# yunfanye/Bittorrent-with-Congestion-Control

Hardware: AMD Instinct MI355X
Metric: GiB/s SHA-1 hashed (device-resident 512KiB chunks) at 1/2/4/8 MI355X (higher is better)
Workload: dtype u32

## Files before the change

### bittorrent-with-congestion-control_amd/btsha1.py

```python
import ctypes
import os

HERE = os.path.dirname(os.path.abspath(__file__))
LIB_PATH = os.environ.get("BT_SHA1_LIB", os.path.join(HERE, "libbtsha1.so"))
CHUNK = 512 * 1024
DIGEST = 20


class BtSha1Error(RuntimeError):
    pass


if not os.path.exists(LIB_PATH):
    raise ImportError(f"libbtsha1.so not built at {LIB_PATH}: run `make` (or __graft_entry__.build())")
lib = ctypes.CDLL(LIB_PATH)

_u8p = ctypes.POINTER(ctypes.c_uint8)
_vp = ctypes.c_void_p
_u64 = ctypes.c_uint64
_i64 = ctypes.c_int64


class Verdict(ctypes.Structure):
    _fields_ = [("tag", ctypes.c_uint64), ("ok", ctypes.c_int32), ("digest", ctypes.c_uint8 * 20)]
# ... 31 lines not shown
_sig("bt_sha1_last_error", ctypes.c_char_p)
_sig("bt_sha1_build_info", ctypes.c_char_p)
_sig("bt_sha1_set_ring_depth", ctypes.c_int, ctypes.c_int)
_sig("bt_sha1_set_variant", ctypes.c_int, ctypes.c_int, ctypes.c_int, ctypes.c_int)
_sig("bt_sha1_set_latency_batch", _u64, _u64)
_sig("bt_sha1_set_seglist_latency_batch", _u64, _u64)
_sig("bt_sha1_seglist_kernel_name", ctypes.c_char_p, _u64)
_sig("bt_sha1_chunks_dev", ctypes.c_int, _vp, _u64, _u64, _u64, _vp, _vp)
_sig("bt_sha1_verify_dev", ctypes.c_int, _vp, _u64, _u64, _u64, _vp, _vp, _vp, _vp)
_sig("bt_sha1_column_dev", ctypes.c_int, _vp, _u64, _u64, _u64, ctypes.c_int, _vp, _u64, _vp, _vp, _vp, _vp)
_sig("bt_sha1_ragged_dev", ctypes.c_int, _vp, _vp, _vp, _u64, _vp, _vp)
_sig("bt_sha1_ragged_verify_dev", ctypes.c_int, _vp, _vp, _vp, _u64, _vp, _vp, _vp, _vp)
_sig("bt_sha1_fill_synthetic", ctypes.c_int, _vp, _u64, _u64, _u64, _vp)
_sig("bt_sha1_chunks_host", _i64, _vp, _u64, _u64, _vp)
_sig("bt_sha1_host_register", ctypes.c_int, _vp, _u64)
_sig("bt_sha1_host_unregister", ctypes.c_int, _vp)
_sig("bt_sha1_chunks_host_multi", _i64, _vp, _u64, _u64, _vp, ctypes.c_int)
_sig("bt_sha1_chunks_host_devices", _i64, _vp, _u64, _u64, _vp, ctypes.POINTER(ctypes.c_int), ctypes.c_int)
_sig("bt_sha1_source_id", ctypes.c_char_p)
_sig("bt_sha1_set_chain_batch", _u64, _u64)
_sig("bt_sha1_kernel_name", ctypes.c_char_p, _u64)
_sig("bt_sha1_clock_probe", ctypes.c_int, _vp, _u64, _u64, _u64, _vp, _vp, _vp)
_sig("bt_sha1_wallclock_khz", _i64)
_sig("bt_sha1_debug_barrier_stats", ctypes.c_int, ctypes.POINTER(ctypes.c_uint64), ctypes.c_int)
_sig("bt_sha1_debug_dropin_residue", _i64, ctypes.c_int)
_sig("bt_sha1_chunks_file", _i64, _vp, _u64, _vp, _u64)
_sig("bt_sha1_get_pipeline_stats", ctypes.c_int, ctypes.POINTER(PipelineStats))
_sig("bt_sha1_set_pageable_feed", ctypes.c_int, ctypes.c_int)
_sig("bt_sha1_verifier_create", _vp, ctypes.c_int, ctypes.c_uint32, ctypes.c_uint32, ctypes.c_uint32)
_sig("bt_sha1_verifier_destroy", None, _vp)
_sig("bt_sha1_verifier_slot", _vp, _vp)
_sig("bt_sha1_verifier_commit", ctypes.c_int, _vp, _vp, ctypes.c_uint32, _vp, _u64)
_sig("bt_sha1_verifier_release", ctypes.c_int, _vp, _vp)
_sig("bt_sha1_verifier_submit", ctypes.c_int, _vp, _vp, ctypes.c_uint32, _vp, _u64)
_sig("bt_sha1_verifier_flush", ctypes.c_int, _vp)
_sig("bt_sha1_verifier_poll", ctypes.c_int, _vp, ctypes.POINTER(Verdict), ctypes.c_int)
_sig("bt_sha1_verifier_drain", ctypes.c_int, _vp, ctypes.POINTER(Verdict), ctypes.c_int)
_sig("bt_sha1_verifier_pending", _i64, _vp)


class VerifierStats(ctypes.Structure):
    _fields_ = [(f, ctypes.c_uint64) for f in ("batches", "ragged_batches", "chunks", "short_chunks", "released")]


_sig("bt_sha1_verifier_create_ragged", _vp, ctypes.c_int, ctypes.c_uint32, ctypes.c_uint32, ctypes.c_uint32)
_sig("bt_sha1_verifier_get_stats", ctypes.c_int, _vp, ctypes.POINTER(VerifierStats))


class Seg(ctypes.Structure):
    _fields_ = [("off", ctypes.c_uint64), ("len", ctypes.c_uint32), ("reserved", ctypes.c_uint32)]


class VerifierGatherStats(ctypes.Structure):
    _fields_ = [(f, ctypes.c_uint64) for f in ("gather_batches", "gather_chunks", "segments", "payload_bytes",
                                               "copied_bytes")]


_sig("bt_sha1_gather_dev", ctypes.c_int, _vp, _vp, _vp, _vp, _u64, _vp, _vp)
_sig("bt_sha1_gather_verify_dev", ctypes.c_int, _vp, _vp, _vp, _vp, _u64, _vp, _vp, _vp, _vp)
_sig("bt_sha1_set_segchain_batch", _u64, _u64)


class PktGeom(ctypes.Structure):
    _fields_ = [(f, ctypes.c_uint32) for f in ("stride", "header", "payload", "slot_pkts")]


# ... 400 lines not shown
            self.h = lib.bt_sha1_verifier_create_gather(device, chunk_len, max_segs, batch, nstreams)
        else:
            create = lib.bt_sha1_verifier_create_ragged if ragged else lib.bt_sha1_verifier_create
            self.h = create(device, chunk_len, batch, nstreams)
        if not self.h:
            kind = "_gather" if gather else "_ragged" if ragged else ""
            raise BtSha1Error(f"bt_sha1_verifier_create{kind}: {last_error()}")
        self.chunk_len = chunk_len
        self.ragged = ragged
        self.gather = gather
        self.max_segs = max_segs

    def submit(self, chunk, expected, tag):
        buf, n = _host_buf(chunk)
        e = (ctypes.c_uint8 * 20).from_buffer_copy(bytes(expected))
        _check(lib.bt_sha1_verifier_submit(self.h, buf, n, e, tag), "bt_sha1_verifier_submit")

    def slot(self):
        p = lib.bt_sha1_verifier_slot(self.h)
        if not p:
            raise BtSha1Error(f"bt_sha1_verifier_slot: {last_error()}")
        return p

    def commit(self, slot, expected, tag, length=None):
        e = (ctypes.c_uint8 * 20).from_buffer_copy(bytes(expected))
        _check(lib.bt_sha1_verifier_commit(self.h, slot, length or self.chunk_len, e, tag),
               "bt_sha1_verifier_commit")

    def commit_gather(self, slot, segs, expected, tag):
        e = (ctypes.c_uint8 * 20).from_buffer_copy(bytes(expected))
        table = (Seg * max(len(segs), 1))(*[Seg(off, length, 0) for off, length in segs])
        _check(lib.bt_sha1_verifier_commit_gather(self.h, slot, table, len(segs), e, tag),
               "bt_sha1_verifier_commit_gather")

    def release(self, slot):
        _check(lib.bt_sha1_verifier_release(self.h, slot), "bt_sha1_verifier_release")

    def flush(self):
        _check(lib.bt_sha1_verifier_flush(self.h), "bt_sha1_verifier_flush")

    def slot_fill(self, chunk, expected, tag):
        p = self.slot()
        ctypes.memmove(p, bytes(chunk), len(chunk))
        self.commit(p, expected, tag, len(chunk))

    def _collect(self, fn, max_n=4096):
        out = (Verdict * max_n)()
        got = _check(fn(self.h, out, max_n), "verifier")
        return [(out[i].tag, bool(out[i].ok), bytes(out[i].digest)) for i in range(got)]

    def poll(self):
        return self._collect(lib.bt_sha1_verifier_poll)

    def drain(self):
        res = []
        while True:
            r = self._collect(lib.bt_sha1_verifier_drain)
            if not r:
                return res
            res += r

    def pending(self):
        return lib.bt_sha1_verifier_pending(self.h)

    def stats(self):
        s = VerifierStats()
# ... 230 lines not shown
```

### bittorrent-with-congestion-control_amd/csrc/bt_runtime.cpp

```cpp
#include "bt_runtime.h"

#include <cstdarg>
#include <memory>
#include <vector>

namespace btsha1 {

thread_local std::string t_err;
__thread int t_dev = 0;
std::atomic<int> g_variant{310};

void set_err(const char *fmt, ...) {
  char buf[512];
  va_list ap;
  va_start(ap, fmt);
  vsnprintf(buf, sizeof buf, fmt, ap);
  va_end(ap);
  t_err = buf;
}

[[noreturn]] void die(const char *where) {
  fprintf(stderr, "libbtsha1: %s: %s\n", where, t_err.c_str());
  fflush(stderr);
  abort();
}

bool trace_on() {
  static const bool on = [] {
    const char *e = getenv("BT_SHA1_TRACE");
    return e && *e && *e != '0';
  }();
  return on;
}

namespace {
std::mutex g_ctx_mu;
std::vector<std::unique_ptr<DevCtx>> g_ctx;
}

int device_count() {
  int n = 0;
  if (hipGetDeviceCount(&n) != hipSuccess) return 0;
  return n;
}

DevCtx *ctx_for(int dev) {
  std::lock_guard<std::mutex> g(g_ctx_mu);
  int n = device_count();
  if (n <= 0) {
    set_err("no HIP device visible (hipGetDeviceCount = 0)");
    return nullptr;
// ... 593 lines not shown
```

### bittorrent-with-congestion-control_amd/csrc/bt_runtime.h

```cpp
#pragma once
#include <hip/hip_runtime.h>

#include <algorithm>
#include <atomic>
#include <chrono>
#include <cstdio>
#include <cstdlib>
#include <cstring>
#include <functional>
#include <mutex>
#include <string>

#include <sched.h>

#include "bt_sha1.h"
#include "sha1_launch.h"

namespace btsha1 __attribute__((visibility("hidden"))) {

extern thread_local std::string t_err;
extern __thread int t_dev;
extern std::atomic<int> g_variant;

void set_err(const char *fmt, ...);

#define BT_CK(expr)                                                                  \
  do {                                                                               \
    hipError_t e_ = (expr);                                                          \
    if (e_ != hipSuccess) {                                                          \
      set_err("%s failed: %s (%s:%d)", #expr, hipGetErrorString(e_), __FILE__, __LINE__); \
      return -1;                                                                     \
    }                                                                                \
  } while (0)

[[noreturn]] void die(const char *where);

struct KeepDevice {
  int prev = -1;
  KeepDevice() {
    if (hipGetDevice(&prev) != hipSuccess) prev = -1;
  }
  ~KeepDevice() {
    int cur = -1;
    if (prev >= 0 && hipGetDevice(&cur) == hipSuccess && cur != prev) (void)hipSetDevice(prev);
  }
  KeepDevice(const KeepDevice &) = delete;
  KeepDevice &operator=(const KeepDevice &) = delete;
};

constexpr uint32_t kMaxColumns = 16;

struct DevBuf {
  void *p = nullptr;
  size_t cap = 0;
  int ensure(size_t need) {
    if (need <= cap) return 0;
    if (p) (void)hipFree(p);
    p = nullptr;
    cap = 0;
    size_t sz = std::max<size_t>(need, 4096);
    BT_CK(hipMalloc(&p, sz));
    cap = sz;
    return 0;
  }
  void release() {
// ... 99 lines not shown
```

### bittorrent-with-congestion-control_amd/csrc/bt_verifier.cpp

```cpp
#include "bt_columns.h"
#include "bt_runtime.h"

#include <deque>
#include <vector>

using namespace btsha1;

struct VBatch {
  hipStream_t s = nullptr;
  hipEvent_t ev = nullptr;
  hipStream_t hs = nullptr;
  hipEvent_t cev[kMaxColumns] = {};
  uint32_t *d_state = nullptr;
  StageBuf slots;
  uint8_t *h_in = nullptr, *h_exp = nullptr, *h_ok = nullptr, *h_dig = nullptr;
  uint64_t *h_off = nullptr;
  uint32_t *h_len = nullptr;
  bt_sha1_seg *h_segs = nullptr;
  uint64_t *h_first = nullptr;
  uint32_t *h_count = nullptr;
  uint8_t *d_in = nullptr;
  std::vector<uint64_t> tags;
  std::vector<uint8_t> state;
  uint32_t reserved = 0, settled = 0;
  bool closed = false, inflight = false;
};

struct bt_sha1_verifier {
  int dev = 0;
  uint32_t chunk_len = 0, batch = 0;
  uint32_t pitch = 0;
  bool ragged = false;
  bool gather = false;
  uint32_t max_segs = 0;
  bt_sha1_verifier_stats st = {};
  bt_sha1_verifier_gather_stats gs = {};
  std::vector<VBatch> b;
  uint32_t fill = 0;
  std::deque<uint32_t> order;
  std::deque<bt_sha1_verdict> done;
  int64_t queued = 0;
};

namespace {

int v_harvest(bt_sha1_verifier *v, VBatch &b) {
  BT_CK(hipEventSynchronize(b.ev));
  for (uint32_t i = 0; i < b.reserved; ++i) {
    if (b.state[i] != 2) continue;
    bt_sha1_verdict r;
    r.tag = b.tags[i];
    r.ok = b.h_ok[i] ? 1 : 0;
    memcpy(r.digest, b.h_dig + 20 * i, 20);
    v->done.push_back(r);
  }
  std::fill(b.state.begin(), b.state.end(), 0);
  b.reserved = b.settled = 0;
  b.closed = b.inflight = false;
  return 0;
}

uint32_t v_columns(uint64_t chunk_len, uint64_t rows) {
  const uint32_t parts = split_columns(chunk_len);
  return parts && rows >= 2 && rows * chunk_len >= column_min_bytes() ? parts : 0;
}

int v_launch_columns(bt_sha1_verifier *v, VBatch &b, uint32_t parts) {
  const uint64_t cl = v->chunk_len, rows = b.reserved, w = cl / parts;
  if (!b.hs) BT_CK(hipStreamCreateWithFlags(&b.hs, hipStreamNonBlocking));
  if (!b.d_state) BT_CK(hipMalloc((void **)&b.d_state, 20 * (size_t)v->batch));
  const ColumnRun run{b.s, b.hs, b.cev, parts, rows, w, cl, b.d_in, b.d_state};
  for (uint32_t j = 0; j < parts; ++j) {
    BT_CK(hipMemcpy2DAsync(b.d_in + j * rows * w, (size_t)w, b.h_in + j * w, (size_t)cl, (size_t)w, (size_t)rows,
                           hipMemcpyHostToDevice, b.s));
    const bool last = j + 1 == parts;
    if (hash_column(run, j, last ? b.h_dig : nullptr, last ? b.h_exp : nullptr, last ? b.h_ok : nullptr)) return -1;
  }
  BT_CK(hipEventRecord(b.ev, b.hs));
  return 0;
}

bool v_needs_ragged(const bt_sha1_verifier *v, const VBatch &b) {
  if (!v->ragged) return false;
  if (v->pitch != v->chunk_len) return true;
  for (uint32_t i = 0; i < b.reserved; ++i)
    if (b.state[i] == 2 && b.h_len[i] != v->chunk_len) return true;
  return false;
}

int v_launch(bt_sha1_verifier *v, uint32_t idx) {
  VBatch &b = v->b[idx];
  if (b.reserved == 0) {
    b.closed = false;
    return 0;
  }
  ++v->st.batches;
  if (v->gather) {
    const size_t bytes = (size_t)b.reserved * v->pitch;
    ++v->gs.gather_batches;
    v->gs.copied_bytes += bytes;
    BT_CK(hipMemcpyAsync(b.d_in, b.h_in, bytes, hipMemcpyHostToDevice, b.s));
    BT_CK(btsha1_launch_gather(b.d_in, b.h_segs, b.h_first, b.h_count, b.reserved, b.h_dig, b.h_exp, b.h_ok, b.s));
    BT_CK(hipEventRecord(b.ev, b.s));
    b.inflight = true;
    v->order.push_back(idx);
    return 0;
  }
  if (v_needs_ragged(v, b)) {
    ++v->st.ragged_batches;
    BT_CK(hipMemcpyAsync(b.d_in, b.h_in, (size_t)b.reserved * v->pitch, hipMemcpyHostToDevice, b.s));
    BT_CK(btsha1_launch_ragged_verify(b.d_in, b.h_off, b.h_len, 0, 0, b.reserved, b.h_dig, b.h_exp, b.h_ok, b.s));
    BT_CK(hipEventRecord(b.ev, b.s));
    b.inflight = true;
    v->order.push_back(idx);
    return 0;
  }
  if (const uint32_t parts = v_columns(v->chunk_len, b.reserved)) {
    if (v_launch_columns(v, b, parts)) {
      if (b.s) (void)hipStreamSynchronize(b.s);
      if (b.hs) (void)hipStreamSynchronize(b.hs);
      return -1;
    }
    b.inflight = true;
    v->order.push_back(idx);
    return 0;
  }
  const size_t bytes = (size_t)b.reserved * v->chunk_len;
  BT_CK(hipMemcpyAsync(b.d_in, b.h_in, bytes, hipMemcpyHostToDevice, b.s));
  BT_CK(btsha1_launch_fixed(b.d_in, b.reserved, v->chunk_len, v->chunk_len, b.h_dig, b.h_exp, b.h_ok, b.s,
                            g_variant.load()));
  BT_CK(hipEventRecord(b.ev, b.s));
  b.inflight = true;
  v->order.push_back(idx);
  return 0;
}

int v_maybe_launch(bt_sha1_verifier *v, uint32_t idx) {
  VBatch &b = v->b[idx];
  if (b.closed && !b.inflight && b.settled == b.reserved) return v_launch(v, idx);
  return 0;
}

int v_advance(bt_sha1_verifier *v) {
  const uint32_t nxt = (v->fill + 1) % (uint32_t)v->b.size();
  VBatch &n = v->b[nxt];
  if (n.inflight) {
    while (!v->order.empty()) {
      const uint32_t o = v->order.front();
      v->order.pop_front();
      if (v_harvest(v, v->b[o])) return -1;
      if (o == nxt) break;
    }
  } else if (n.closed) {
    set_err("verifier: every batch holds slots that were handed out but never committed");
    return -1;
  }
  v->fill = nxt;
  return 0;
}

int v_locate(bt_sha1_verifier *v, const uint8_t *slot, uint32_t *bi, uint32_t *si) {
  for (uint32_t k = 0; k < v->b.size(); ++k) {
    VBatch &b = v->b[k];
    if (slot >= b.h_in && slot < b.h_in + (size_t)v->batch * v->pitch) {
      const size_t off = (size_t)(slot - b.h_in);
      if (off % v->pitch || b.state[off / v->pitch] != 1) break;
      *bi = k;
      *si = (uint32_t)(off / v->pitch);
      return 0;
    }
  }
  set_err("verifier: pointer is not an outstanding slot");
  return -1;
}

int v_check_len(const bt_sha1_verifier *v, uint32_t len) {
  if (v->gather) {
    if (len == 0 || len > v->chunk_len) {
      set_err("verifier: chunk of %u bytes, gather verifier's slots take 1 .. %u", len, v->chunk_len);
      return -1;
    }
  } else if (v->ragged) {
    if (len == 0 || len > v->chunk_len) {
      set_err("verifier: chunk of %u bytes, ragged verifier takes 1 .. %u", len, v->chunk_len);
      return -1;
    }
  } else if (len != v->chunk_len) {
    set_err("verifier: chunk of %u bytes, verifier built for %u", len, v->chunk_len);
    return -1;
  }
  return 0;
}

bt_sha1_verifier *v_create(int device, uint32_t chunk_len, uint32_t batch, uint32_t nstreams, bool ragged,
                           uint32_t max_segs = 0) {
  const bool gather = max_segs != 0;
  DevCtx *c = ctx_for(device);
  if (!c) return nullptr;
  KeepDevice keep_dev;
  if (hipSetDevice(device) != hipSuccess) {
    set_err("hipSetDevice(%d) failed", device);
    return nullptr;
  }
  int node = -1;
  {
    std::lock_guard<std::mutex> g(c->mu);
    if (c->numa_node == -2) c->numa_node = gpu_numa_node(device);
    node = placement_for(c->numa_node).node;
  }
  auto *v = new bt_sha1_verifier;
  v->dev = device;
  v->chunk_len = chunk_len;
  v->pitch = ragged || gather ? (chunk_len + 15u) & ~15u : chunk_len;
  v->ragged = ragged;
  v->gather = gather;
  v->max_segs = max_segs;
  v->batch = batch;
  v->b.resize(std::max<uint32_t>(nstreams, 2));
  const size_t bytes = (size_t)batch * v->pitch;
  t_err.clear();
  for (auto &b : v->b) {
    b.tags.resize(batch);
    b.state.assign(batch, 0);
    if (hipStreamCreateWithFlags(&b.s, hipStreamNonBlocking) != hipSuccess ||
        hipEventCreateWithFlags(&b.ev, hipEventDisableTiming) != hipSuccess ||
        b.slots.ensure(bytes, node) != 0 ||
        hipHostMalloc((void **)&b.h_exp, 20 * (size_t)batch, hipHostMallocDefault) != hipSuccess ||
        hipHostMalloc((void **)&b.h_ok, batch, hipHostMallocDefault) != hipSuccess ||
        hipHostMalloc((void **)&b.h_dig, 20 * (size_t)batch, hipHostMallocDefault) != hipSuccess ||
        hipMalloc((void **)&b.d_in, bytes) != hipSuccess ||
        (ragged && (hipHostMalloc((void **)&b.h_off, 8 * (size_t)batch, hipHostMallocDefault) != hipSuccess ||
                    hipHostMalloc((void **)&b.h_len, 4 * (size_t)batch, hipHostMallocDefault) != hipSuccess)) ||
        (gather &&
         (hipHostMalloc((void **)&b.h_segs, sizeof(bt_sha1_seg) * (size_t)batch * max_segs, hipHostMallocDefault) !=
              hipSuccess ||
          hipHostMalloc((void **)&b.h_first, 8 * (size_t)batch, hipHostMallocDefault) != hipSuccess ||
          hipHostMalloc((void **)&b.h_count, 4 * (size_t)batch, hipHostMallocDefault) != hipSuccess))) {
      if (t_err.empty()) set_err("verifier: allocation failed");
      bt_sha1_verifier_destroy(v);
      return nullptr;
    }
    b.h_in = b.slots.as<uint8_t>();
    for (uint32_t i = 0; ragged && i < batch; ++i) {
      b.h_off[i] = (uint64_t)i * v->pitch;
      b.h_len[i] = 0;
    }
    for (uint32_t i = 0; gather && i < batch; ++i) {
      b.h_first[i] = (uint64_t)i * max_segs;
      b.h_count[i] = 0;
    }
  }
  return v;
}

}

extern "C" {

bt_sha1_verifier *bt_sha1_verifier_create(int device, uint32_t chunk_len, uint32_t batch, uint32_t nstreams) {
// ... 59 lines not shown
  v->gs.segments += nseg;
  v->gs.payload_bytes += payload;
  ++v->st.chunks;
  b.tags[si] = tag;
  b.state[si] = 2;
  ++b.settled;
  ++v->queued;
  return v_maybe_launch(v, bi);
}

int bt_sha1_verifier_get_gather_stats(bt_sha1_verifier *v, bt_sha1_verifier_gather_stats *out) {
  if (!v || !out) {
    set_err("null pointer");
    return -1;
  }
  *out = v->gs;
  return 0;
}

void bt_sha1_verifier_destroy(bt_sha1_verifier *v) {
  if (!v) return;
  KeepDevice keep_dev;
  (void)hipSetDevice(v->dev);
  for (auto &b : v->b) {
    if (b.s) (void)hipStreamSynchronize(b.s);
    if (b.hs) (void)hipStreamSynchronize(b.hs);
    if (b.ev) (void)hipEventDestroy(b.ev);
    for (hipEvent_t e : b.cev)
      if (e) (void)hipEventDestroy(e);
    if (b.s) (void)hipStreamDestroy(b.s);
    if (b.hs) (void)hipStreamDestroy(b.hs);
    if (b.d_state) (void)hipFree(b.d_state);
    b.slots.release();
    if (b.h_exp) (void)hipHostFree(b.h_exp);
    if (b.h_ok) (void)hipHostFree(b.h_ok);
    if (b.h_dig) (void)hipHostFree(b.h_dig);
    if (b.h_off) (void)hipHostFree(b.h_off);
    if (b.h_len) (void)hipHostFree(b.h_len);
    if (b.h_segs) (void)hipHostFree(b.h_segs);
    if (b.h_first) (void)hipHostFree(b.h_first);
    if (b.h_count) (void)hipHostFree(b.h_count);
    if (b.d_in) (void)hipFree(b.d_in);
  }
  delete v;
}

uint8_t *bt_sha1_verifier_slot(bt_sha1_verifier *v) {
  if (!v) return nullptr;
  KeepDevice keep_dev;
  if (hipSetDevice(v->dev) != hipSuccess) return nullptr;
  if (v->b[v->fill].closed && v_advance(v)) return nullptr;
  VBatch &b = v->b[v->fill];
  const uint32_t j = b.reserved++;
  b.state[j] = 1;
  if (b.reserved == v->batch) b.closed = true;
  return b.h_in + (size_t)j * v->pitch;
}

int bt_sha1_verifier_commit(bt_sha1_verifier *v, uint8_t *slot, uint32_t len, const uint8_t expected[20],
                            uint64_t tag) {
  if (!v || !slot || !expected) {
    set_err("null pointer");
    return -1;
  }
  if (v_check_len(v, len)) return -1;
  KeepDevice keep_dev;
  if (hipSetDevice(v->dev) != hipSuccess) return -1;
  uint32_t bi, si;
  if (v_locate(v, slot, &bi, &si)) return -1;
  VBatch &b = v->b[bi];
  memcpy(b.h_exp + 20 * (size_t)si, expected, 20);
  if (v->ragged) b.h_len[si] = len;
  if (v->gather) {
    b.h_segs[(size_t)si * v->max_segs] = bt_sha1_seg{(uint64_t)si * v->pitch, len, 0};
    b.h_count[si] = 1;
    ++v->gs.gather_chunks;
    ++v->gs.segments;
    v->gs.payload_bytes += len;
  }
  ++v->st.chunks;
  if (!v->gather && len < v->chunk_len) ++v->st.short_chunks;
  b.tags[si] = tag;
  b.state[si] = 2;
  ++b.settled;
  ++v->queued;
  return v_maybe_launch(v, bi);
}

int bt_sha1_verifier_release(bt_sha1_verifier *v, uint8_t *slot) {
  if (!v || !slot) {
    set_err("null pointer");
    return -1;
  }
  KeepDevice keep_dev;
  if (hipSetDevice(v->dev) != hipSuccess) return -1;
  uint32_t bi, si;
  if (v_locate(v, slot, &bi, &si)) return -1;
  VBatch &b = v->b[bi];
  memset(b.h_exp + 20 * (size_t)si, 0, 20);
  if (v->ragged) b.h_len[si] = 0;
  if (v->gather) b.h_count[si] = 0;
  ++v->st.released;
  b.state[si] = 3;
  ++b.settled;
  return v_maybe_launch(v, bi);
}

int bt_sha1_verifier_submit(bt_sha1_verifier *v, const void *h_chunk, uint32_t len, const uint8_t expected[20],
                            uint64_t tag) {
  if (!v || !h_chunk) {
    set_err("null pointer");
    return -1;
  }
  if (v_check_len(v, len)) return -1;
  uint8_t *slot = bt_sha1_verifier_slot(v);
  if (!slot) return -1;
  memcpy(slot, h_chunk, len);
  return bt_sha1_verifier_commit(v, slot, len, expected, tag);
}

int bt_sha1_verifier_flush(bt_sha1_verifier *v) {
  if (!v) return -1;
  KeepDevice keep_dev;
  if (hipSetDevice(v->dev) != hipSuccess) return -1;
  VBatch &b = v->b[v->fill];
  if (b.reserved == 0 || b.closed) return 0;
  b.closed = true;
  return v_maybe_launch(v, v->fill);
}

static int v_take(bt_sha1_verifier *v, bt_sha1_verdict *out, int max) {
  int n = 0;
  while (n < max && !v->done.empty()) {
    out[n++] = v->done.front();
    v->done.pop_front();
  }
  v->queued -= n;
  return n;
}

int bt_sha1_verifier_poll(bt_sha1_verifier *v, bt_sha1_verdict *out, int max) {
  if (!v) return -1;
  KeepDevice keep_dev;
  if (hipSetDevice(v->dev) != hipSuccess) return -1;
  while (!v->order.empty()) {
    VBatch &b = v->b[v->order.front()];
    hipError_t q = hipEventQuery(b.ev);
    if (q == hipErrorNotReady) break;
    if (q != hipSuccess) {
      set_err("verifier: %s", hipGetErrorString(q));
      return -1;
    }
    v->order.pop_front();
    if (v_harvest(v, b)) return -1;
  }
  return v_take(v, out, max);
}

int bt_sha1_verifier_drain(bt_sha1_verifier *v, bt_sha1_verdict *out, int max) {
  if (!v) return -1;
  if (bt_sha1_verifier_flush(v)) return -1;
  while (!v->order.empty()) {
    const uint32_t o = v->order.front();
    v->order.pop_front();
    if (v_harvest(v, v->b[o])) return -1;
  }
  return v_take(v, out, max);
}

int64_t bt_sha1_verifier_pending(bt_sha1_verifier *v) { return v ? v->queued : -1; }

int bt_sha1_verifier_get_stats(bt_sha1_verifier *v, bt_sha1_verifier_stats *out) {
  if (!v || !out) {
    set_err("null pointer");
    return -1;
  }
  *out = v->st;
  return 0;
}

}
```

### bittorrent-with-congestion-control_amd/host/verify_stream.c

```c
#include <fcntl.h>
#include <pthread.h>
#include <stdio.h>
#include <stdlib.h>
#include <string.h>
#include <sys/mman.h>
#include <sys/stat.h>
#include <time.h>
#include <unistd.h>

#include "bt_sha1.h"
#include "chunk.h"

#define PAYLOAD 1484
#define PACKET 1500
#define HEADER (PACKET - PAYLOAD)
#define MAX_DGRAMS ((BT_CHUNK_SIZE + PAYLOAD - 1) / PAYLOAD)
#define GATHER_SLOT ((MAX_DGRAMS + 1) * PACKET)
#define ARRIVAL_WINDOW 8

static void count(const bt_sha1_verdict *out, int m, long *good, long *bad) {
  for (int i = 0; i < m; i++) {
    if (out[i].ok) {
      (*good)++;
    } else {
// ... 14 lines not shown
static int cmp_resident(const void *a, const void *b) {
  const struct resident *x = (const struct resident *)a, *y = (const struct resident *)b;
  if (x->slot != y->slot) return x->slot < y->slot ? -1 : 1;
  return x->seq < y->seq ? -1 : x->seq > y->seq;
}

static int cmp_slot(const void *a, const void *b) {
  const uint8_t *x = ((const struct resident *)a)->slot, *y = ((const struct resident *)b)->slot;
  return x < y ? -1 : x > y;
}

static long index_resident(struct resident *res, long nres) {
  qsort(res, nres, sizeof *res, cmp_resident);
  long m = 0;
  for (long i = 0; i < nres; i++) {
    if (m && res[m - 1].slot == res[i].slot) m--;
    res[m++] = res[i];
  }
  return m;
}

static double now(void) {
  struct timespec ts;
  clock_gettime(CLOCK_MONOTONIC, &ts);
  return ts.tv_sec + 1e-9 * ts.tv_nsec;
}

struct shared {
  const uint8_t *img;
  const int *ids;
  const uint8_t *exp;
  const uint32_t *len;
  int corrupt, zcopy, gather, poll_every, rounds, warm;
  long ring;
  pthread_barrier_t *bar;
  double *t0;
};

struct lane {
  bt_sha1_verifier *v;
  int *ks;
  int nk;
  long per_round;
  struct resident *res;
  long nres;
  long good, bad, total, timed, late_fills, commits, segments;
  uint64_t timed_bytes, wire_bytes;
  int err;
  const struct shared *sh;
};

static int drain_lane(struct lane *l, int wait) {
  bt_sha1_verdict out[256];
  int m;
  while ((m = wait ? bt_sha1_verifier_drain(l->v, out, 256) : bt_sha1_verifier_poll(l->v, out, 256)) > 0)
    count(out, m, &l->good, &l->bad);
  if (m < 0) {
    fprintf(stderr, "verify-stream: %s\n", bt_sha1_last_error());
    return -1;
  }
  return 0;
}

static uint32_t next_rand(uint32_t *x) {
  *x = *x * 1664525u + 1013904223u;
  return *x >> 8;
// ... 66 lines not shown
      l->res[at].k = k;
      l->nres++;
      fill = 1;
      if (r >= sh->warm) l->late_fills++;
    } else {
      fprintf(stderr, "verify-stream: more distinct slots than the ring holds (%p)\n", (void *)slot);
      return -1;
    }
  }
  if (sh->gather) {
    const uint32_t clen = sh->len[k], landed = (clen + PAYLOAD - 1) / PAYLOAD + 1;
    if (r == 0 || fill)
      land_datagrams(slot, sh->img + (uint64_t)sh->ids[k] * BT_CHUNK_SIZE, clen, k,
                     sh->corrupt && k % 7 == 3 ? (long)(k % clen) : -1);
    bt_sha1_seg segs[MAX_DGRAMS];
    const uint32_t nseg = list_segments(slot, landed, segs);
    if (nseg != landed - 1) {
      fprintf(stderr, "verify-stream -G: chunk %d: %u sequence numbers in %u datagrams\n", k, nseg, landed);
      return -1;
    }
    if (bt_sha1_verifier_commit_gather(l->v, slot, segs, nseg, sh->exp + 20 * k, (uint64_t)k)) {
      fprintf(stderr, "verify-stream: %s\n", bt_sha1_last_error());
      return -1;
    }
    if (r >= sh->warm) {
      l->segments += nseg;
      l->wire_bytes += (uint64_t)landed * PACKET;
    }
  } else if (!sh->zcopy || r == 0 || fill) {
    const uint64_t off = (uint64_t)sh->ids[k] * BT_CHUNK_SIZE;
    const uint32_t clen = sh->len[k];
    for (uint32_t got = 0; got < clen; got += PAYLOAD) {
      uint32_t len = clen - got < PAYLOAD ? clen - got : PAYLOAD;
      memcpy(slot + got, sh->img + off + got, len);
    }
    if (sh->corrupt && k % 7 == 3) slot[k % clen] ^= 0x5a;
  }
  if (!sh->gather && bt_sha1_verifier_commit(l->v, slot, sh->len[k], sh->exp + 20 * k, (uint64_t)k)) {
    fprintf(stderr, "verify-stream: %s\n", bt_sha1_last_error());
    return -1;
  }
  l->total++;
  if (r >= sh->warm) {
    l->timed++;
    l->timed_bytes += sh->len[k];
  }
  if (++l->commits % sh->poll_every == 0 && drain_lane(l, 0)) return -1;
  return 0;
}

static int round_end(struct lane *l, int r) {
  const struct shared *sh = l->sh;
  if (r + 1 == sh->warm && drain_lane(l, 1)) return -1;
  if (sh->zcopy && r == 0) l->nres = index_resident(l->res, l->nres);
  return 0;
}

static void *lane_thread(void *arg) {
  struct lane *l = (struct lane *)arg;
  const struct shared *sh = l->sh;
  for (int r = 0; r < sh->rounds; r++) {
    for (long i = 0; i < l->per_round && !l->err; i++)
      if (receive_one(l, r, i)) l->err = 1;
    if (!l->err && round_end(l, r)) l->err = 1;
    if (r + 1 == sh->warm) {
      if (pthread_barrier_wait(sh->bar) == PTHREAD_BARRIER_SERIAL_THREAD) *sh->t0 = now();
      pthread_barrier_wait(sh->bar);
    }
  }
  if (!l->err && drain_lane(l, 1)) l->err = 1;
  return NULL;
}

#define USAGE \
  "usage: %s [-b batch] [-s streams] [-r rounds] [-w warmup-rounds] [-p poll-every] [-g verifiers] [-t] [-x] [-z | -G [-c]] " \
  "<data-file> <chunks-file>\n"

int main(int argc, char **argv) {
  int batch = 64, streams = 2, rounds = 1, corrupt = 0, zcopy = 0, poll_every = 1, G = 1, threads = 0, warm = 0, opt;
  int gather = 0, segchain = 0;
  while ((opt = getopt(argc, argv, "b:s:r:w:p:g:txzGc")) != -1) {
    if (opt == 'b') batch = atoi(optarg);
    else if (opt == 's') streams = atoi(optarg);
    else if (opt == 'r') rounds = atoi(optarg);
    else if (opt == 'w') warm = atoi(optarg);
    else if (opt == 'x') corrupt = 1;
    else if (opt == 'z') zcopy = 1;
    else if (opt == 'G') gather = 1;
    else if (opt == 'c') segchain = 1;
    else if (opt == 't') threads = 1;
    else if (opt == 'p') poll_every = atoi(optarg) > 0 ? atoi(optarg) : 1;
    else if (opt == 'g') G = atoi(optarg);
    else {
      fprintf(stderr, USAGE, argv[0]);
      return 255;
    }
  }
  if (gather && zcopy) {
    fprintf(stderr, "verify-stream: -z and -G are two receive models, take one\n");
    return 255;
  }
  if (segchain && !gather) {
    fprintf(stderr, "verify-stream: -c selects the kernel of -G's segment lists, it needs -G\n");
    return 255;
  }
  const int resident = zcopy || gather;
  if (argc - optind != 2 || G < 1 || G > 64 || rounds < 1 || warm < 0 || batch < 1) {
    fprintf(stderr, USAGE, argv[0]);
    return 255;
  }
  if (resident && rounds > 1 && warm < 1) warm = 1;
  if (warm >= rounds) {
    fprintf(stderr, "verify-stream: -w %d leaves no timed round of %d\n", warm, rounds);
    return 255;
  }
  int fd = open(argv[optind], O_RDONLY);
  struct stat st;
  if (fd < 0 || fstat(fd, &st) != 0) {
    perror(argv[optind]);
    return 255;
  }
  const uint8_t *img = st.st_size ? (const uint8_t *)mmap(NULL, st.st_size, PROT_READ, MAP_PRIVATE, fd, 0) : NULL;
// ... 9 lines not shown
  while (fgets(line, sizeof line, cf)) {
    int id;
    if (line[0] == '#' || sscanf(line, "%d %127s", &id, hex) != 2 || strlen(hex) != 40) continue;
    if (n == cap) {
      cap *= 2;
      ids = realloc(ids, sizeof(int) * cap);
      exp = realloc(exp, 20 * cap);
    }
    ids[n] = id;
    hex2binary(hex, 40, exp + 20 * n);
    n++;
  }
  fclose(cf);

  uint32_t *clen = malloc(sizeof(uint32_t) * (n ? n : 1));
  int m0 = 0, any_short = 0;
  for (int k = 0; k < n; k++)
    if (ids[k] >= 0 && (uint64_t)ids[k] * BT_CHUNK_SIZE < (uint64_t)st.st_size) {
      const uint64_t left = (uint64_t)st.st_size - (uint64_t)ids[k] * BT_CHUNK_SIZE;
      ids[m0] = ids[k];
      memcpy(exp + 20 * m0, exp + 20 * k, 20);
      clen[m0] = left < BT_CHUNK_SIZE ? (uint32_t)left : BT_CHUNK_SIZE;
      if (clen[m0] < BT_CHUNK_SIZE) any_short = 1;
      m0++;
    }
  n = m0;
  const int ndev = bt_sha1_device_count();
  if (ndev <= 0) {
    fprintf(stderr, "verify-stream: no HIP device visible\n");
    return 255;
  }
  double t0 = 0;
  pthread_barrier_t bar;
  struct shared sh = {img, ids, exp, clen, corrupt, resident, gather, poll_every, rounds, warm,
                      (long)batch * (streams < 2 ? 2 : streams), &bar, &t0};
  struct lane *L = calloc((size_t)G, sizeof *L);
  if (segchain) bt_sha1_set_segchain_batch(UINT64_MAX);
  long per_round_max = 0;
  for (int g = 0; g < G; g++) {
    L[g].sh = &sh;
    L[g].v = gather ? bt_sha1_verifier_create_gather(g % ndev, GATHER_SLOT, MAX_DGRAMS, (uint32_t)batch,
                                                     (uint32_t)streams)
             : any_short ? bt_sha1_verifier_create_ragged(g % ndev, BT_CHUNK_SIZE, (uint32_t)batch, (uint32_t)streams)
                       : bt_sha1_verifier_create(g % ndev, BT_CHUNK_SIZE, (uint32_t)batch, (uint32_t)streams);
    if (!L[g].v) {
      fprintf(stderr, "verify-stream: %s\n", bt_sha1_last_error());
      return 255;
    }
    L[g].ks = malloc(sizeof(int) * (n ? n : 1));
    for (int k = 0; k < n; k++)
      if (ids[k] % G == g) L[g].ks[L[g].nk++] = k;
    L[g].per_round = L[g].nk;
    if (resident) {
      if (L[g].nk == 0 || sh.ring % L[g].nk) {
        fprintf(stderr, "verify-stream %s: batch*streams (%ld) must be a multiple of each verifier's chunk count "
                        "(verifier %d: %d)\n", gather ? "-G" : "-z", sh.ring, g, L[g].nk);
        return 255;
      }
      L[g].per_round = sh.ring;
      L[g].res = malloc(sizeof *L[g].res * sh.ring);
    }
    if (L[g].per_round > per_round_max) per_round_max = L[g].per_round;
  }
  int err = 0;
  t0 = now();
  if (threads && G > 1) {
    pthread_barrier_init(&bar, NULL, (unsigned)G);
// ... 12 lines not shown
      for (int g = 0; g < G && !err; g++)
        if (round_end(&L[g], r)) err = 1;
      if (r + 1 == warm) t0 = now();
    }
    for (int g = 0; g < G && !err; g++)
      if (drain_lane(&L[g], 1)) err = 1;
  }
  if (err) return 255;
  double dt = now() - t0;
  long good = 0, bad = 0, total = 0, timed = 0, late = 0;
  uint64_t timed_bytes = 0, wire_bytes = 0;
  long segments = 0;
  for (int g = 0; g < G; g++) {
    segments += L[g].segments;
    wire_bytes += L[g].wire_bytes;
    good += L[g].good;
    bad += L[g].bad;
    total += L[g].total;
    timed += L[g].timed;
    timed_bytes += L[g].timed_bytes;
    late += L[g].late_fills;
    bt_sha1_verifier_destroy(L[g].v);
    free(L[g].ks);
    free(L[g].res);
  }
  free(L);
  free(clen);
  printf("{\"chunks\": %ld, \"ok\": %ld, \"failed\": %ld, \"seconds\": %.6f, \"GiB_per_s\": %.4f, \"batch\": %d, "
         "\"streams\": %d, \"poll_every\": %d, \"verifiers\": %d, \"devices\": %d, \"receive_threads\": %d, "
         "\"rounds\": %d, \"warmup_rounds\": %d, \"timed_chunks\": %ld, \"late_fills\": %ld, \"mode\": \"%s\"",
         total, good, bad, dt, (double)timed_bytes / dt / (1u << 30), batch, streams, poll_every, G,
         G < ndev ? G : ndev, threads ? G : 1, rounds, warm, timed, late,
         gather ? "datagram slots" : zcopy ? "zero-copy slots" : "packetized memcpy (util.c:275)");
  if (gather)
    printf(", \"segments\": %ld, \"hashed_bytes\": %llu, \"wire_bytes\": %llu", segments,
           (unsigned long long)timed_bytes, (unsigned long long)wire_bytes);
  if (segchain) printf(", \"segchain\": true");
  printf("}\n");
  return bad && !corrupt ? 1 : 0;
}
```

### include/bt_sha1.h

```cpp
#ifndef BT_SHA1_H
#define BT_SHA1_H

#include <stddef.h>
#include <stdint.h>

#include "sha.h"

#ifdef __cplusplus
extern "C" {
#endif

#define BT_SHA1_DIGEST_SIZE 20

int bt_sha1_device_count(void);
int bt_sha1_set_device(int device);
const char *bt_sha1_last_error(void);
const char *bt_sha1_build_info(void);
const char *bt_sha1_source_id(void);
int bt_sha1_set_ring_depth(int nbuf);
int bt_sha1_set_variant(int nbuf, int lines, int nt);
uint64_t bt_sha1_set_latency_batch(uint64_t max_chunks);
uint64_t bt_sha1_set_chain_batch(uint64_t max_messages);
uint64_t bt_sha1_set_seglist_latency_batch(uint64_t max_messages);
uint64_t bt_sha1_set_segchain_batch(uint64_t max_messages);
// ... 90 lines not shown
  int32_t copy_threads;
  int32_t numa_nodes;
  int32_t gpu_numa_node;
  int32_t numa_policy;
  int32_t registered_batches;
  uint32_t column_chunks;
  double total_s;
  double alloc_s;
  double fill_s;
  double wait_s;
  double register_s;
  double unregister_s;
  int32_t lane_pages[BT_SHA1_STATS_NODES];
  int32_t src_pages[BT_SHA1_STATS_NODES];
  int32_t copy_pieces[BT_SHA1_STATS_NODES];
} bt_sha1_pipeline_stats;
int bt_sha1_get_pipeline_stats(bt_sha1_pipeline_stats *out);

typedef struct bt_sha1_verifier bt_sha1_verifier;
typedef struct {
  uint64_t tag;
  int32_t ok;
  uint8_t digest[BT_SHA1_DIGEST_SIZE];
} bt_sha1_verdict;

bt_sha1_verifier *bt_sha1_verifier_create(int device, uint32_t chunk_len, uint32_t batch,
                                          uint32_t nstreams);
bt_sha1_verifier *bt_sha1_verifier_create_ragged(int device, uint32_t max_chunk_len, uint32_t batch,
                                                 uint32_t nstreams);
void bt_sha1_verifier_destroy(bt_sha1_verifier *v);
uint8_t *bt_sha1_verifier_slot(bt_sha1_verifier *v);
int bt_sha1_verifier_commit(bt_sha1_verifier *v, uint8_t *slot, uint32_t len,
                            const uint8_t expected[20], uint64_t tag);
int bt_sha1_verifier_release(bt_sha1_verifier *v, uint8_t *slot);
int bt_sha1_verifier_submit(bt_sha1_verifier *v, const void *h_chunk, uint32_t len,
                            const uint8_t expected[20], uint64_t tag);
int bt_sha1_verifier_flush(bt_sha1_verifier *v);
int bt_sha1_verifier_poll(bt_sha1_verifier *v, bt_sha1_verdict *out, int max);
int bt_sha1_verifier_drain(bt_sha1_verifier *v, bt_sha1_verdict *out, int max);
int64_t bt_sha1_verifier_pending(bt_sha1_verifier *v);
typedef struct {
  uint64_t batches;
  uint64_t ragged_batches;
  uint64_t chunks;
  uint64_t short_chunks;
  uint64_t released;
} bt_sha1_verifier_stats;
int bt_sha1_verifier_get_stats(bt_sha1_verifier *v, bt_sha1_verifier_stats *out);
bt_sha1_verifier *bt_sha1_verifier_create_gather(int device, uint32_t slot_len, uint32_t max_segs,
                                                 uint32_t batch, uint32_t nstreams);
int bt_sha1_verifier_commit_gather(bt_sha1_verifier *v, uint8_t *slot, const bt_sha1_seg *segs,
                                   uint32_t nseg, const uint8_t expected[20], uint64_t tag);
typedef struct {
  uint64_t gather_batches;
  uint64_t gather_chunks;
  uint64_t segments;
  uint64_t payload_bytes;
  uint64_t copied_bytes;
} bt_sha1_verifier_gather_stats;
int bt_sha1_verifier_get_gather_stats(bt_sha1_verifier *v, bt_sha1_verifier_gather_stats *out);

typedef struct bt_sha1_receiver bt_sha1_receiver;
bt_sha1_receiver *bt_sha1_receiver_create(int device, uint32_t chunk_len, uint32_t nslots,
                                          uint32_t stride);
void bt_sha1_receiver_destroy(bt_sha1_receiver *r);
uint8_t *bt_sha1_receiver_slot(bt_sha1_receiver *r);
// ... 84 lines not shown
```

Baseline: 3277.

## Add streaming-store slot writer API for verifier packet fills

Adds bt_sha1_verifier_write, which copies packet payloads into pinned slot memory using non-temporal SSE stores, with a per-slot 64-byte carry line for unaligned tails that is flushed at commit or release. The verify-stream harness now uses it by default instead of memcpy, with -m restoring the old memcpy path. It also replaces the deque batch order with a fixed ring array and outlines the BT_CK error path to shrink hot code. The aim is to avoid cache pollution and read-for-ownership traffic on host writes into pinned buffers that the GPU DMA then reads. The cost is an extra per-call slot lookup and carry bookkeeping for each small write.

Result: no change. 3263 (-0.4%).

```diff
diff --git a/bittorrent-with-congestion-control_amd/btsha1.py b/bittorrent-with-congestion-control_amd/btsha1.py
--- a/bittorrent-with-congestion-control_amd/btsha1.py
+++ b/bittorrent-with-congestion-control_amd/btsha1.py
@@ -87,6 +87,7 @@
 _sig("bt_sha1_verifier_slot", _vp, _vp)
 _sig("bt_sha1_verifier_commit", ctypes.c_int, _vp, _vp, ctypes.c_uint32, _vp, _u64)
 _sig("bt_sha1_verifier_release", ctypes.c_int, _vp, _vp)
+_sig("bt_sha1_verifier_write", ctypes.c_int, _vp, _vp, ctypes.c_uint32, _vp, ctypes.c_uint32)
 _sig("bt_sha1_verifier_submit", ctypes.c_int, _vp, _vp, ctypes.c_uint32, _vp, _u64)
 _sig("bt_sha1_verifier_flush", ctypes.c_int, _vp)
 _sig("bt_sha1_verifier_poll", ctypes.c_int, _vp, ctypes.POINTER(Verdict), ctypes.c_int)
@@ -553,6 +554,10 @@
         table = (Seg * max(len(segs), 1))(*[Seg(off, length, 0) for off, length in segs])
         _check(lib.bt_sha1_verifier_commit_gather(self.h, slot, table, len(segs), e, tag),
                "bt_sha1_verifier_commit_gather")
+
+    def write(self, slot, offset, payload):
+        buf, n = _host_buf(payload)
+        _check(lib.bt_sha1_verifier_write(self.h, slot, offset, buf, n), "bt_sha1_verifier_write")
 
     def release(self, slot):
         _check(lib.bt_sha1_verifier_release(self.h, slot), "bt_sha1_verifier_release")
diff --git a/bittorrent-with-congestion-control_amd/csrc/bt_runtime.cpp b/bittorrent-with-congestion-control_amd/csrc/bt_runtime.cpp
--- a/bittorrent-with-congestion-control_amd/csrc/bt_runtime.cpp
+++ b/bittorrent-with-congestion-control_amd/csrc/bt_runtime.cpp
@@ -17,6 +17,11 @@
   vsnprintf(buf, sizeof buf, fmt, ap);
   va_end(ap);
   t_err = buf;
+}
+
+int ck_failed(hipError_t e, const char *expr, const char *file, int line) {
+  set_err("%s failed: %s (%s:%d)", expr, hipGetErrorString(e), file, line);
+  return -1;
 }
 
 [[noreturn]] void die(const char *where) {
diff --git a/bittorrent-with-congestion-control_amd/csrc/bt_runtime.h b/bittorrent-with-congestion-control_amd/csrc/bt_runtime.h
--- a/bittorrent-with-congestion-control_amd/csrc/bt_runtime.h
+++ b/bittorrent-with-congestion-control_amd/csrc/bt_runtime.h
@@ -24,13 +24,12 @@
 
 void set_err(const char *fmt, ...);
 
+int ck_failed(hipError_t e, const char *expr, const char *file, int line);
+
 #define BT_CK(expr)                                                                  \
   do {                                                                               \
     hipError_t e_ = (expr);                                                          \
-    if (e_ != hipSuccess) {                                                          \
-      set_err("%s failed: %s (%s:%d)", #expr, hipGetErrorString(e_), __FILE__, __LINE__); \
-      return -1;                                                                     \
-    }                                                                                \
+    if (e_ != hipSuccess) return ck_failed(e_, #expr, __FILE__, __LINE__);           \
   } while (0)
 
 [[noreturn]] void die(const char *where);
diff --git a/bittorrent-with-congestion-control_amd/csrc/bt_slotwrite.h b/bittorrent-with-congestion-control_amd/csrc/bt_slotwrite.h
--- /dev/null
+++ b/bittorrent-with-congestion-control_amd/csrc/bt_slotwrite.h
@@ -0,0 +1,76 @@
+#pragma once
+
+#include <cassert>
+#include <cstdint>
+#include <cstring>
+
+#if defined(__x86_64__)
+#include <emmintrin.h>
+#endif
+
+struct SlotCarry {
+  uint8_t line[64];
+  uint64_t at;
+  uint32_t have;
+};
+
+#if defined(__x86_64__)
+
+static inline void slot_flush(uint8_t *slot, SlotCarry &c) {
+  if (c.have) {
+    memcpy(slot + (c.at - c.have), c.line, c.have);
+    c.have = 0;
+  }
+  _mm_sfence();
+}
+
+static inline void slot_stream_line(uint8_t *dst, const uint8_t *src) {
+  const __m128i a = _mm_loadu_si128((const __m128i *)src), b = _mm_loadu_si128((const __m128i *)(src + 16)),
+                c = _mm_loadu_si128((const __m128i *)(src + 32)), d = _mm_loadu_si128((const __m128i *)(src + 48));
+  _mm_stream_si128((__m128i *)dst, a);
+  _mm_stream_si128((__m128i *)(dst + 16), b);
+  _mm_stream_si128((__m128i *)(dst + 32), c);
+  _mm_stream_si128((__m128i *)(dst + 48), d);
+}
+
+static inline void slot_write(uint8_t *slot, SlotCarry &c, uint64_t off, const void *src, uint32_t len) {
+  assert(((uintptr_t)slot & 63) == 0);
+  const uint8_t *s = (const uint8_t *)src;
+  if (off != c.at || (c.have == 0 && (off & 63))) {
+    slot_flush(slot, c);
+    const uint32_t to_line = (uint32_t)(-off & 63), head = len < to_line ? len : to_line;
+    memcpy(slot + off, s, head);
+    s += head;
+    len -= head;
+    c.at = off + head;
+  }
+  if (c.have) {
+    const uint32_t need = 64 - c.have, take = len < need ? len : need;
+    memcpy(c.line + c.have, s, take);
+    s += take;
+    len -= take;
+    c.at += take;
+    c.have += take;
+    if (c.have < 64) return;
+    slot_stream_line(slot + (c.at - 64), c.line);
+    c.have = 0;
+  }
+  uint8_t *d = slot + c.at;
+  c.at += len;
+  for (; len >= 64; len -= 64, s += 64, d += 64) {
+    _mm_prefetch((const char *)s + 256, _MM_HINT_NTA);
+    slot_stream_line(d, s);
+  }
+  memcpy(c.line, s, len);
+  c.have = len;
+}
+
+#else
+
+static inline void slot_flush(uint8_t *, SlotCarry &) {}
+
+static inline void slot_write(uint8_t *slot, SlotCarry &, uint64_t off, const void *src, uint32_t len) {
+  memcpy(slot + off, src, len);
+}
+
+#endif
diff --git a/bittorrent-with-congestion-control_amd/csrc/bt_verifier.cpp b/bittorrent-with-congestion-control_amd/csrc/bt_verifier.cpp
--- a/bittorrent-with-congestion-control_amd/csrc/bt_verifier.cpp
+++ b/bittorrent-with-congestion-control_amd/csrc/bt_verifier.cpp
@@ -1,5 +1,6 @@
 #include "bt_columns.h"
 #include "bt_runtime.h"
+#include "bt_slotwrite.h"
 
 #include <deque>
 #include <vector>
@@ -22,6 +23,7 @@
   uint8_t *d_in = nullptr;
   std::vector<uint64_t> tags;
   std::vector<uint8_t> state;
+  SlotCarry *carry = nullptr;
   uint32_t reserved = 0, settled = 0;
   bool closed = false, inflight = false;
 };
@@ -37,14 +39,24 @@
   bt_sha1_verifier_gather_stats gs = {};
   std::vector<VBatch> b;
   uint32_t fill = 0;
-  std::deque<uint32_t> order;
+  uint32_t *order = nullptr;
+  uint32_t ohead = 0, norder = 0;
+  void order_push(uint32_t idx) { order[(ohead + norder++) % b.size()] = idx; }
+  uint32_t order_pop() {
+    const uint32_t o = order[ohead];
+    ohead = (ohead + 1) % (uint32_t)b.size();
+    --norder;
+    return o;
+  }
   std::deque<bt_sha1_verdict> done;
   int64_t queued = 0;
+  const uint8_t *w_slot = nullptr;
+  uint32_t w_bi = 0, w_si = 0;
 };
 
 namespace {
 
-int v_harvest(bt_sha1_verifier *v, VBatch &b) {
+__attribute__((noinline)) int v_harvest(bt_sha1_verifier *v, VBatch &b) {
   BT_CK(hipEventSynchronize(b.ev));
   for (uint32_t i = 0; i < b.reserved; ++i) {
     if (b.state[i] != 2) continue;
@@ -95,43 +107,32 @@
     return 0;
   }
   ++v->st.batches;
-  if (v->gather) {
-    const size_t bytes = (size_t)b.reserved * v->pitch;
-    ++v->gs.gather_batches;
-    v->gs.copied_bytes += bytes;
-    BT_CK(hipMemcpyAsync(b.d_in, b.h_in, bytes, hipMemcpyHostToDevice, b.s));
-    BT_CK(btsha1_launch_gather(b.d_in, b.h_segs, b.h_first, b.h_count, b.reserved, b.h_dig, b.h_exp, b.h_ok, b.s));
-    BT_CK(hipEventRecord(b.ev, b.s));
-    b.inflight = true;
-    v->order.push_back(idx);
-    return 0;
-  }
-  if (v_needs_ragged(v, b)) {
-    ++v->st.ragged_batches;
-    BT_CK(hipMemcpyAsync(b.d_in, b.h_in, (size_t)b.reserved * v->pitch, hipMemcpyHostToDevice, b.s));
-    BT_CK(btsha1_launch_ragged_verify(b.d_in, b.h_off, b.h_len, 0, 0, b.reserved, b.h_dig, b.h_exp, b.h_ok, b.s));
-    BT_CK(hipEventRecord(b.ev, b.s));
-    b.inflight = true;
-    v->order.push_back(idx);
-    return 0;
-  }
-  if (const uint32_t parts = v_columns(v->chunk_len, b.reserved)) {
+  const bool ragged = !v->gather && v_needs_ragged(v, b);
+  const uint32_t parts = v->gather || ragged ? 0 : v_columns(v->chunk_len, b.reserved);
+  if (parts) {
     if (v_launch_columns(v, b, parts)) {
       if (b.s) (void)hipStreamSynchronize(b.s);
       if (b.hs) (void)hipStreamSynchronize(b.hs);
       return -1;
     }
-    b.inflight = true;
-    v->order.push_back(idx);
-    return 0;
-  }
-  const size_t bytes = (size_t)b.reserved * v->chunk_len;
-  BT_CK(hipMemcpyAsync(b.d_in, b.h_in, bytes, hipMemcpyHostToDevice, b.s));
-  BT_CK(btsha1_launch_fixed(b.d_in, b.reserved, v->chunk_len, v->chunk_len, b.h_dig, b.h_exp, b.h_ok, b.s,
-                            g_variant.load()));
-  BT_CK(hipEventRecord(b.ev, b.s));
+  } else {
+    const size_t bytes = (size_t)b.reserved * v->pitch;
+    BT_CK(hipMemcpyAsync(b.d_in, b.h_in, bytes, hipMemcpyHostToDevice, b.s));
+    if (v->gather) {
+      ++v->gs.gather_batches;
+      v->gs.copied_bytes += bytes;
+      BT_CK(btsha1_launch_gather(b.d_in, b.h_segs, b.h_first, b.h_count, b.reserved, b.h_dig, b.h_exp, b.h_ok, b.s));
+    } else if (ragged) {
+      ++v->st.ragged_batches;
+      BT_CK(btsha1_launch_ragged_verify(b.d_in, b.h_off, b.h_len, 0, 0, b.reserved, b.h_dig, b.h_exp, b.h_ok, b.s));
+    } else {
+      BT_CK(btsha1_launch_fixed(b.d_in, b.reserved, v->chunk_len, v->chunk_len, b.h_dig, b.h_exp, b.h_ok, b.s,
+                                g_variant.load()));
+    }
+    BT_CK(hipEventRecord(b.ev, b.s));
+  }
   b.inflight = true;
-  v->order.push_back(idx);
+  v->order_push(idx);
   return 0;
 }
 
@@ -145,9 +146,8 @@
   const uint32_t nxt = (v->fill + 1) % (uint32_t)v->b.size();
   VBatch &n = v->b[nxt];
   if (n.inflight) {
-    while (!v->order.empty()) {
-      const uint32_t o = v->order.front();
-      v->order.pop_front();
+    while (v->norder) {
+      const uint32_t o = v->order_pop();
       if (v_harvest(v, v->b[o])) return -1;
       if (o == nxt) break;
     }
@@ -174,6 +174,12 @@
   return -1;
 }
 
+__attribute__((noinline)) void v_settle_writes(bt_sha1_verifier *v, VBatch &b, const uint8_t *slot, uint32_t si) {
+  slot_flush(b.h_in, b.carry[si]);
+  b.carry[si].at = 0;
+  if (v->w_slot == slot) v->w_slot = nullptr;
+}
+
 int v_check_len(const bt_sha1_verifier *v, uint32_t len) {
   if (v->gather) {
     if (len == 0 || len > v->chunk_len) {
@@ -217,14 +223,15 @@
   v->max_segs = max_segs;
   v->batch = batch;
   v->b.resize(std::max<uint32_t>(nstreams, 2));
+  v->order = (uint32_t *)calloc(v->b.size(), sizeof(uint32_t));
   const size_t bytes = (size_t)batch * v->pitch;
   t_err.clear();
   for (auto &b : v->b) {
     b.tags.resize(batch);
     b.state.assign(batch, 0);
-    if (hipStreamCreateWithFlags(&b.s, hipStreamNonBlocking) != hipSuccess ||
+    if (!v->order || hipStreamCreateWithFlags(&b.s, hipStreamNonBlocking) != hipSuccess ||
         hipEventCreateWithFlags(&b.ev, hipEventDisableTiming) != hipSuccess ||
-        b.slots.ensure(bytes, node) != 0 ||
+        b.slots.ensure(bytes, node) != 0 || !(b.carry = (SlotCarry *)calloc(batch, sizeof(SlotCarry))) ||
         hipHostMalloc((void **)&b.h_exp, 20 * (size_t)batch, hipHostMallocDefault) != hipSuccess ||
         hipHostMalloc((void **)&b.h_ok, batch, hipHostMallocDefault) != hipSuccess ||
         hipHostMalloc((void **)&b.h_dig, 20 * (size_t)batch, hipHostMallocDefault) != hipSuccess ||
@@ -350,6 +357,7 @@
     if (b.hs) (void)hipStreamDestroy(b.hs);
     if (b.d_state) (void)hipFree(b.d_state);
     b.slots.release();
+    free(b.carry);
     if (b.h_exp) (void)hipHostFree(b.h_exp);
     if (b.h_ok) (void)hipHostFree(b.h_ok);
     if (b.h_dig) (void)hipHostFree(b.h_dig);
@@ -360,6 +368,7 @@
     if (b.h_count) (void)hipHostFree(b.h_count);
     if (b.d_in) (void)hipFree(b.d_in);
   }
+  free(v->order);
   delete v;
 }
 
@@ -387,6 +396,7 @@
   uint32_t bi, si;
   if (v_locate(v, slot, &bi, &si)) return -1;
   VBatch &b = v->b[bi];
+  v_settle_writes(v, b, slot, si);
   memcpy(b.h_exp + 20 * (size_t)si, expected, 20);
   if (v->ragged) b.h_len[si] = len;
   if (v->gather) {
@@ -405,6 +415,25 @@
   return v_maybe_launch(v, bi);
 }
 
+int bt_sha1_verifier_write(bt_sha1_verifier *v, uint8_t *slot, uint32_t offset, const void *src, uint32_t len) {
+  if (!v || !slot || !src) {
+    set_err("null pointer");
+    return -1;
+  }
+  if (slot != v->w_slot) {
+    if (v_locate(v, slot, &v->w_bi, &v->w_si)) return -1;
+    v->w_slot = slot;
+  }
+  if (v->gather || (uint64_t)offset + len > v->chunk_len) {
+    set_err("verifier: write of %u bytes at %u: past the slot's %u bytes, or a gather verifier's slot", len, offset,
+            v->chunk_len);
+    return -1;
+  }
+  VBatch &b = v->b[v->w_bi];
+  slot_write(b.h_in, b.carry[v->w_si], (uint64_t)v->w_si * v->pitch + offset, src, len);
+  return 0;
+}
+
 int bt_sha1_verifier_release(bt_sha1_verifier *v, uint8_t *slot) {
   if (!v || !slot) {
     set_err("null pointer");
@@ -415,6 +444,7 @@
   uint32_t bi, si;
   if (v_locate(v, slot, &bi, &si)) return -1;
   VBatch &b = v->b[bi];
+  v_settle_writes(v, b, slot, si);
   memset(b.h_exp + 20 * (size_t)si, 0, 20);
   if (v->ragged) b.h_len[si] = 0;
   if (v->gather) b.h_count[si] = 0;
@@ -461,15 +491,15 @@
   if (!v) return -1;
   KeepDevice keep_dev;
   if (hipSetDevice(v->dev) != hipSuccess) return -1;
-  while (!v->order.empty()) {
-    VBatch &b = v->b[v->order.front()];
+  while (v->norder) {
+    VBatch &b = v->b[v->order[v->ohead]];
     hipError_t q = hipEventQuery(b.ev);
     if (q == hipErrorNotReady) break;
     if (q != hipSuccess) {
       set_err("verifier: %s", hipGetErrorString(q));
       return -1;
     }
-    v->order.pop_front();
+    v->order_pop();
     if (v_harvest(v, b)) return -1;
   }
   return v_take(v, out, max);
@@ -478,11 +508,8 @@
 int bt_sha1_verifier_drain(bt_sha1_verifier *v, bt_sha1_verdict *out, int max) {
   if (!v) return -1;
   if (bt_sha1_verifier_flush(v)) return -1;
-  while (!v->order.empty()) {
-    const uint32_t o = v->order.front();
-    v->order.pop_front();
-    if (v_harvest(v, v->b[o])) return -1;
-  }
+  while (v->norder)
+    if (v_harvest(v, v->b[v->order_pop()])) return -1;
   return v_take(v, out, max);
 }
 
diff --git a/bittorrent-with-congestion-control_amd/host/verify_stream.c b/bittorrent-with-congestion-control_amd/host/verify_stream.c
--- a/bittorrent-with-congestion-control_amd/host/verify_stream.c
+++ b/bittorrent-with-congestion-control_amd/host/verify_stream.c
@@ -70,6 +70,7 @@
   const uint8_t *exp;
   const uint32_t *len;
   int corrupt, zcopy, gather, poll_every, rounds, warm;
+  int plain;
   long ring;
   pthread_barrier_t *bar;
   double *t0;
@@ -202,9 +203,22 @@
     const uint32_t clen = sh->len[k];
     for (uint32_t got = 0; got < clen; got += PAYLOAD) {
       uint32_t len = clen - got < PAYLOAD ? clen - got : PAYLOAD;
-      memcpy(slot + got, sh->img + off + got, len);
-    }
-    if (sh->corrupt && k % 7 == 3) slot[k % clen] ^= 0x5a;
+      if (sh->plain) {
+        memcpy(slot + got, sh->img + off + got, len);
+      } else if (bt_sha1_verifier_write(l->v, slot, got, sh->img + off + got, len)) {
+        fprintf(stderr, "verify-stream: %s\n", bt_sha1_last_error());
+        return -1;
+      }
+    }
+    if (sh->corrupt && k % 7 == 3) {
+      const uint8_t flipped = sh->img[off + k % clen] ^ 0x5a;
+      if (sh->plain) {
+        slot[k % clen] = flipped;
+      } else if (bt_sha1_verifier_write(l->v, slot, k % clen, &flipped, 1)) {
+        fprintf(stderr, "verify-stream: %s\n", bt_sha1_last_error());
+        return -1;
+      }
+    }
   }
   if (!sh->gather && bt_sha1_verifier_commit(l->v, slot, sh->len[k], sh->exp + 20 * k, (uint64_t)k)) {
     fprintf(stderr, "verify-stream: %s\n", bt_sha1_last_error());
@@ -243,13 +257,13 @@
 }
 
 #define USAGE \
-  "usage: %s [-b batch] [-s streams] [-r rounds] [-w warmup-rounds] [-p poll-every] [-g verifiers] [-t] [-x] [-z | -G [-c]] " \
+  "usage: %s [-b batch] [-s streams] [-r rounds] [-w warmup-rounds] [-p poll-every] [-g verifiers] [-t] [-x] [-m] [-z | -G [-c]] " \
   "<data-file> <chunks-file>\n"
 
 int main(int argc, char **argv) {
   int batch = 64, streams = 2, rounds = 1, corrupt = 0, zcopy = 0, poll_every = 1, G = 1, threads = 0, warm = 0, opt;
-  int gather = 0, segchain = 0;
-  while ((opt = getopt(argc, argv, "b:s:r:w:p:g:txzGc")) != -1) {
+  int gather = 0, segchain = 0, plain = 0;
+  while ((opt = getopt(argc, argv, "b:s:r:w:p:g:txzGcm")) != -1) {
     if (opt == 'b') batch = atoi(optarg);
     else if (opt == 's') streams = atoi(optarg);
     else if (opt == 'r') rounds = atoi(optarg);
@@ -258,6 +272,7 @@
     else if (opt == 'z') zcopy = 1;
     else if (opt == 'G') gather = 1;
     else if (opt == 'c') segchain = 1;
+    else if (opt == 'm') plain = 1;
     else if (opt == 't') threads = 1;
     else if (opt == 'p') poll_every = atoi(optarg) > 0 ? atoi(optarg) : 1;
     else if (opt == 'g') G = atoi(optarg);
@@ -333,7 +348,7 @@
   }
   double t0 = 0;
   pthread_barrier_t bar;
-  struct shared sh = {img, ids, exp, clen, corrupt, resident, gather, poll_every, rounds, warm,
+  struct shared sh = {img, ids, exp, clen, corrupt, resident, gather, poll_every, rounds, warm, plain,
                       (long)batch * (streams < 2 ? 2 : streams), &bar, &t0};
   struct lane *L = calloc((size_t)G, sizeof *L);
   if (segchain) bt_sha1_set_segchain_batch(UINT64_MAX);
@@ -412,6 +427,8 @@
          total, good, bad, dt, (double)timed_bytes / dt / (1u << 30), batch, streams, poll_every, G,
          G < ndev ? G : ndev, threads ? G : 1, rounds, warm, timed, late,
          gather ? "datagram slots" : zcopy ? "zero-copy slots" : "packetized memcpy (util.c:275)");
+  if (plain && !gather)
+    printf(", \"slot_writer\": \"memcpy\"");
   if (gather)
     printf(", \"segments\": %ld, \"hashed_bytes\": %llu, \"wire_bytes\": %llu", segments,
            (unsigned long long)timed_bytes, (unsigned long long)wire_bytes);
diff --git a/include/bt_sha1.h b/include/bt_sha1.h
--- a/include/bt_sha1.h
+++ b/include/bt_sha1.h
@@ -146,6 +146,8 @@
 uint8_t *bt_sha1_verifier_slot(bt_sha1_verifier *v);
 int bt_sha1_verifier_commit(bt_sha1_verifier *v, uint8_t *slot, uint32_t len,
                             const uint8_t expected[20], uint64_t tag);
+int bt_sha1_verifier_write(bt_sha1_verifier *v, uint8_t *slot, uint32_t offset, const void *src,
+                           uint32_t len);
 int bt_sha1_verifier_release(bt_sha1_verifier *v, uint8_t *slot);
 int bt_sha1_verifier_submit(bt_sha1_verifier *v, const void *h_chunk, uint32_t len,
                             const uint8_t expected[20], uint64_t tag);
```
